# cbg-ethz/LongSom

Measured on AMD Instinct MI355X. Metric: genomic sites/s pileup+call, 10M-read BAM x 5k barcodes, 1/2/4/8 MI355X, higher is better.
Workload: dtype u32

## Files before the change

longsom_amd/csrc/call.hip:

```cpp
#include "lsg_ctx.h"
#include "call_rec.h"
#include "bb_tail.h"
#include <cstdio>
#include <cstring>
#include <cstdlib>
#include <hipcub/hipcub.hpp>

namespace lsg {

enum { CT_CAND = 0, CT_NCAND = 1, CT_HEADS = 4, CT_PASS = 6, CT_LIGHT = 16, CT_HEAVY = 32, CT_QTAIL = 48, CT_DEFER = 64, CT_WORDS = 80 };
struct CallArgs {
    const uint32_t* ne_units; const uint64_t* ne_mask; const uint32_t* ne_rowbase; const int2* ne_geom;
    uint32_t n_ne; int32_t n_ct;
    const uint32_t* rows[LSG_MAX_CELLTYPES]; uint64_t row_cap;
    const uint8_t* const* ref_ptr; const int64_t* contig_len;
    lsg_call_params p;
    double lgc0[2], lgcn[2];
    uint32_t* pass_list;
    const int16_t* tail_table;
    uint32_t* site_cnt; uint32_t* site_off;
    SiteRec* sites; CandCt* cands; uint64_t cand_cap;
    struct TailTask* light; struct TailTask* heavy; uint64_t task_cap;
    unsigned long long* counters;
    uint32_t arena_waves;
// ... 36 lines not shown
    const uint32_t up = n - k + 1;
    return k < up ? k : up;
}

__global__ void k_head_recs(CallArgs a) {
    const uint32_t i = blockIdx.x * blockDim.x + threadIdx.x;
    if (i >= (uint32_t)a.counters[CT_HEADS]) return;
    const uint32_t w = a.heads[i];
    const uint32_t tile = a.ne_units[w] / (uint32_t)a.n_ct;
    uint64_t mask[LSG_MAX_CELLTYPES] = {0, 0, 0, 0};
    uint32_t rbase[LSG_MAX_CELLTYPES] = {0, 0, 0, 0};
    for (uint32_t q = w; q < a.n_ne && q < w + (uint32_t)a.n_ct && a.ne_units[q] / (uint32_t)a.n_ct == tile; ++q) {
        const int ct = (int)(a.ne_units[q] % (uint32_t)a.n_ct);
        mask[ct] = a.ne_mask[q]; rbase[ct] = a.ne_rowbase[q];
    }
    const int2 geom = a.ne_geom[w];
    a.head_ref[i] = (uint64_t)(uintptr_t)a.ref_ptr[geom.y & 0xffffff];
    uint32_t* r = a.head_recs + (uint64_t)i * 16;
    r[0] = (uint32_t)a.contig_len[geom.y & 0xffffff]; r[1] = a.site_off[w]; r[2] = (uint32_t)geom.x; r[3] = (uint32_t)geom.y;
    for (int ct = 0; ct < LSG_MAX_CELLTYPES; ++ct) { r[4 + 2 * ct] = (uint32_t)mask[ct]; r[5 + 2 * ct] = (uint32_t)(mask[ct] >> 32); r[12 + ct] = rbase[ct]; }
}

constexpr int GATHER_WAVES = 4;
constexpr uint32_t CAND_CHUNK = 256, TASK_CHUNK = 64, HEAVY_CHUNK = 16;
template <int NCT>
__global__ __launch_bounds__(GATHER_WAVES * 64) __attribute__((amdgpu_waves_per_eu(NCT <= 2 ? 4 : 3))) void k_call_gather(CallArgs a) {
    const int lane = threadIdx.x & 63;
    const uint32_t wave = (uint32_t)__builtin_amdgcn_readfirstlane((int)(uint32_t)(((uint64_t)blockIdx.x * blockDim.x + threadIdx.x) >> 6));
    const uint32_t n_waves = (uint32_t)(((uint64_t)gridDim.x * blockDim.x) >> 6);
    const uint32_t n_heads = (uint32_t)a.counters[CT_HEADS];
    const uint32_t c_base = n_waves * CAND_CHUNK, l_base = n_waves * TASK_CHUNK, h_base = n_waves * HEAVY_CHUNK;
    uint32_t c_next = wave * CAND_CHUNK, c_end = c_next + CAND_CHUNK;
    uint32_t l_next = wave * TASK_CHUNK, l_end = l_next + TASK_CHUNK, h_next = wave * HEAVY_CHUNK, h_end = h_next + HEAVY_CHUNK;
    uint32_t n_cand_exact = 0;
    typedef uint32_t u32x16 __attribute__((ext_vector_type(16)));
    const __attribute__((address_space(4))) u32x16* H = (const __attribute__((address_space(4))) u32x16*)(uintptr_t)a.head_recs;
    const __attribute__((address_space(4))) uint64_t* HR = (const __attribute__((address_space(4))) uint64_t*)(uintptr_t)a.head_ref;
    u32x16 nxt = {};
    uint64_t ref_nxt = 0;
    if (wave < n_heads) { nxt = H[wave]; ref_nxt = HR[wave]; }
    for (uint32_t hi_ = wave; hi_ < n_heads; hi_ += n_waves) {
    const u32x16 rec = nxt;
    const uint8_t* ref = reinterpret_cast<const uint8_t*>((uintptr_t)ref_nxt);
    if (hi_ + n_waves < n_heads) { nxt = H[hi_ + n_waves]; ref_nxt = HR[hi_ + n_waves]; }
    uint64_t mask[NCT];
    uint32_t rbase[NCT];
    uint64_t any = 0;
#pragma unroll
    for (int ct = 0; ct < NCT; ++ct) { mask[ct] = (uint64_t)rec[4 + 2 * ct] | ((uint64_t)rec[5 + 2 * ct] << 32); rbase[ct] = rec[12 + ct]; any |= mask[ct]; }
    const bool site = (any >> lane) & 1ull;
    const uint64_t below = (1ull << lane) - 1ull;
    const uint64_t idx = (uint64_t)rec[1] + __popcll(any & below);
    const int2 geom = make_int2((int)rec[2], (int)rec[3]);
    const int tid = geom.y & 0xffffff;
    const int64_t pos = (int64_t)geom.x + lane;
    const int64_t clen = (int64_t)rec[0];
    const int64_t gx = (int64_t)geom.x;
    const int64_t xpos = lane < 5 ? gx - 5 + lane : gx + 59 + lane;
    const bool r0_ok = pos < clen, r1_ok = lane < 10 && xpos >= 0 && xpos < clen;
    const uint8_t r0_raw = ref[r0_ok ? pos : 0], r1_raw = ref[r1_ok ? xpos : 0];
    struct __attribute__((packed, aligned(4))) Quad { uint32_t x, y, z, w; };
    Quad q[NCT][4];
#pragma unroll
    for (int ct = 0; ct < NCT; ++ct) {
        const bool has_row = site && ((mask[ct] >> lane) & 1ull);
        const uint64_t row = has_row ? (uint64_t)(rbase[ct] & ~ROW_NARROW) + __popcll(mask[ct] & below) : (uint64_t)lane;
        const bool narrow = has_row && (rbase[ct] & ROW_NARROW);
        const char* R = reinterpret_cast<const char*>(a.rows[ct] + (row >> 6) * ROW_BLOCK_WORDS) + (narrow ? (row & 63) * 8 : (row & 63) * 16);
        const uint32_t stride = narrow ? 512u : 1024u;
#pragma unroll
        for (int k = 0; k < 4; ++k) q[ct][k] = *reinterpret_cast<const Quad*>(R + k * stride);
    }
    const uint8_t r0 = r0_ok ? r0_raw : (uint8_t)0, r1 = r1_ok ? r1_raw : (uint8_t)0;
    const uint8_t refb = site ? r0 : (uint8_t)'N';
    const int rsym = sym_of_ref(refb);
    const lsg_call_params& P = a.p;
    const int order[4] = {0, 1, 3, 2};
    uint32_t v_dp[NCT], v_nc[NCT], v_cc[NCT][6], v_bc[NCT][6];
#pragma unroll
    for (int ct = 0; ct < NCT; ++ct) {
        uint4 q0 = make_uint4(q[ct][0].x, q[ct][0].y, q[ct][0].z, q[ct][0].w), q1 = make_uint4(q[ct][1].x, q[ct][1].y, q[ct][1].z, q[ct][1].w);
        uint4 q2 = make_uint4(q[ct][2].x, q[ct][2].y, q[ct][2].z, q[ct][2].w), q3 = make_uint4(q[ct][3].x, q[ct][3].y, q[ct][3].z, q[ct][3].w);
        if (rbase[ct] & ROW_NARROW) {
            q0 = make_uint4(q0.x & 0xffffu, q0.x >> 16, q0.y & 0xffffu, q0.y >> 16); q1 = make_uint4(q1.x & 0xffffu, q1.x >> 16, q1.y & 0xffffu, q1.y >> 16);
            q2 = make_uint4(q2.x & 0xffffu, q2.x >> 16, q2.y & 0xffffu, q2.y >> 16); q3 = make_uint4(q3.x & 0xffffu, q3.x >> 16, q3.y & 0xffffu, q3.y >> 16);
        }
        v_dp[ct] = q0.x; v_nc[ct] = q0.y;
        v_cc[ct][0] = q0.z; v_cc[ct][1] = q0.w; v_cc[ct][2] = q1.x; v_cc[ct][3] = q1.y; v_cc[ct][4] = q1.z; v_cc[ct][5] = q1.w;
        v_bc[ct][0] = q2.z; v_bc[ct][1] = q2.w; v_bc[ct][2] = q3.x; v_bc[ct][3] = q3.y; v_bc[ct][4] = q3.z; v_bc[ct][5] = q3.w;
    }
    const uint32_t prev0 = (uint32_t)__shfl_up((int)r0, 1), prev1 = (uint32_t)__shfl_up((int)r1, 1), next0 = (uint32_t)__shfl_down((int)r0, 1);
    const uint64_t eq0 = __ballot(lane > 0 && r0 == (uint8_t)prev0), eq1 = __ballot(lane > 0 && lane != 5 && lane < 10 && r1 == (uint8_t)prev1);
    const uint32_t r1_4 = (uint32_t)__builtin_amdgcn_readlane((int)r1, 4), r1_5 = (uint32_t)__builtin_amdgcn_readlane((int)r1, 5);
    const uint32_t r0_0 = (uint32_t)__builtin_amdgcn_readlane((int)r0, 0), r0_63 = (uint32_t)__builtin_amdgcn_readlane((int)r0, 63);
    const uint64_t e_lo = (eq1 & 0x1eull) | ((uint64_t)(r0_0 == r1_4) << 5) | (eq0 << 5);
    const uint64_t e_hi = (eq0 >> 59) | ((uint64_t)(r1_5 == r0_63) << 5) | (((eq1 >> 6) & 0xfull) << 6);
    const uint64_t xlo = (e_lo >> 1) | (e_hi << 63), xhi = e_hi >> 1;
    const uint32_t xw = (uint32_t)((xlo >> lane) | (lane ? xhi << (64 - lane) : 0ull));
    const bool have_ctx = pos >= 5;
    int down_len = (int)((clen - (pos + 1)) < 5 ? (clen - (pos + 1)) : 5);
    if (down_len < 0) down_len = 0;
    const uint32_t ue = xw & 15u;
    const uint32_t de = down_len > 0 ? (xw >> 6) & ((1u << (down_len - 1)) - 1u) : 0u;
    auto longest = [](uint32_t m) { const uint32_t m2 = m & (m >> 1), m3 = m2 & (m >> 2), m4 = m3 & (m >> 3); return (int)((m != 0) + (m2 != 0) + (m3 != 0) + (m4 != 0)); };
    const int up_best = 1 + longest(ue), up_run = 1 + (int)__builtin_clz((((~ue) & 15u) << 28) | (1u << 27));
    const int dn_best = 1 + longest(de), dn_run = 1 + (int)__builtin_ctz((~de) | 16u);
    const uint8_t up4 = lane ? (uint8_t)prev0 : (uint8_t)r1_4, dn0 = lane < 63 ? (uint8_t)next0 : (uint8_t)r1_5;
    bool has_any = false, off_table = false;
    uint32_t n_light = 0, n_heavy = 0;
    int32_t s_alts_bc = 0, s_alts_cc = 0, s_dp = 0, s_nc = 0;
    if (site) {
#pragma unroll
        for (int ct = 0; ct < NCT; ++ct) {
            const uint32_t dp = v_dp[ct], nc = v_nc[ct];
            const bool ok = ((mask[ct] >> lane) & 1ull) && (int)dp >= P.min_cov && (int)nc >= P.min_cells;
            s_dp += ok ? (int32_t)dp : 0; s_nc += ok ? (int32_t)nc : 0;
#pragma unroll
            for (int s = 0; s < 6; ++s) {
                const bool nr = ok && s != rsym;
                const uint32_t b = nr ? v_bc[ct][s] : 0u, c = nr ? v_cc[ct][s] : 0u;
                const bool alt = s < 4 && b > 0;
                has_any |= alt;
                s_alts_bc += alt ? 0 : (int32_t)b; s_alts_cc += alt ? 0 : (int32_t)c;
                s_dp -= alt ? (int32_t)b : 0; s_nc -= alt ? (int32_t)c : 0;
                off_table |= alt && !(tail_in_table(b, dp) && tail_in_table(c, nc));
            }
        }
        if (s_alts_bc > 0) {
            off_table |= s_dp >= 0 && !tail_in_table((uint32_t)s_alts_bc, (uint32_t)s_dp);
            off_table |= s_nc >= 0 && s_alts_cc >= 0 && !tail_in_table((uint32_t)s_alts_cc, (uint32_t)s_nc);
        }
    }
    if (__ballot(off_table)) {
        if (site) {
#pragma unroll
            for (int ct = 0; ct < NCT; ++ct) {
                if (!((mask[ct] >> lane) & 1ull)) continue;
                const uint32_t dp = v_dp[ct], nc = v_nc[ct];
                if (!((int)dp >= P.min_cov && (int)nc >= P.min_cells)) continue;
#pragma unroll
                for (int s = 0; s < 4; ++s) {
                    const uint32_t b = v_bc[ct][s], c = v_cc[ct][s];
                    if (s == rsym || b == 0) continue;
                    if (!tail_in_table(b, dp)) { if (tail_work(b, dp) > 64) ++n_heavy; else ++n_light; }
                    if (!tail_in_table(c, nc)) { if (tail_work(c, nc) > 64) ++n_heavy; else ++n_light; }
                }
            }
            if (s_alts_bc > 0) {
                if (s_dp >= 0 && !tail_in_table((uint32_t)s_alts_bc, (uint32_t)s_dp)) { if (tail_work((uint32_t)s_alts_bc, (uint32_t)s_dp) > 64) ++n_heavy; else ++n_light; }
                if (s_nc >= 0 && s_alts_cc >= 0 && !tail_in_table((uint32_t)s_alts_cc, (uint32_t)s_nc)) { if (tail_work((uint32_t)s_alts_cc, (uint32_t)s_nc) > 64) ++n_heavy; else ++n_light; }
            }
        }
    }
    const unsigned long long cm = __ballot(has_any);
    uint32_t pl = n_light, ph = n_heavy, tot_l = 0, tot_h = 0;
    if (__ballot((n_light | n_heavy) != 0u)) {
        for (int o = 1; o < 64; o <<= 1) { const uint32_t vl = __shfl_up(pl, o), vh = __shfl_up(ph, o); if (lane >= o) { pl += vl; ph += vh; } }
        tot_l = __shfl(pl, 63); tot_h = __shfl(ph, 63);
    }
    const uint32_t n_c = (uint32_t)__popcll(cm);
    n_cand_exact += n_c;
    if (c_next + n_c > c_end) {
        uint32_t nb = 0;
        if (lane == 0) nb = (uint32_t)atomicAdd(&a.counters[CT_CAND], (unsigned long long)CAND_CHUNK) + c_base;
        c_next = (uint32_t)__builtin_amdgcn_readfirstlane((int)nb); c_end = c_next + CAND_CHUNK;
    }
    const uint32_t cbase = c_next; c_next += n_c;
    uint32_t l_old = l_next, l_room = l_end - l_next, l_new = 0;
    if (tot_l > l_room) {
        uint32_t nb = 0;
        if (lane == 0) nb = (uint32_t)atomicAdd(&a.counters[CT_LIGHT], (unsigned long long)TASK_CHUNK * ((tot_l - l_room + TASK_CHUNK - 1) / TASK_CHUNK)) + l_base;
        l_new = (uint32_t)__builtin_amdgcn_readfirstlane((int)nb);
        l_next = l_new + (tot_l - l_room); l_end = l_new + TASK_CHUNK * ((tot_l - l_room + TASK_CHUNK - 1) / TASK_CHUNK);
    } else l_next += tot_l;
    uint32_t h_old = h_next, h_room = h_end - h_next, h_new = 0;
    if (tot_h > h_room) {
        uint32_t nb = 0;
        if (lane == 0) nb = (uint32_t)atomicAdd(&a.counters[CT_HEAVY], (unsigned long long)HEAVY_CHUNK * ((tot_h - h_room + HEAVY_CHUNK - 1) / HEAVY_CHUNK)) + h_base;
        h_new = (uint32_t)__builtin_amdgcn_readfirstlane((int)nb);
        h_next = h_new + (tot_h - h_room); h_end = h_new + HEAVY_CHUNK * ((tot_h - h_room + HEAVY_CHUNK - 1) / HEAVY_CHUNK);
    } else h_next += tot_h;
    if (!site) continue;
    const uint32_t cand = cbase + (uint32_t)__popcll(cm & below);
    uint32_t li = pl - n_light, hi = ph - n_heavy;
    const int16_t* TT = a.tail_table;
    auto table_at = [&](uint32_t k, uint32_t n, int set) { return TT[tail_in_table(k, n) ? (uint32_t)set * TAIL_ENTRIES + tail_index(k, n) : 0u]; };
    int16_t t_bc[NCT][4], t_cc[NCT][4];
#pragma unroll
    for (int ct = 0; ct < NCT; ++ct) {
#pragma unroll
        for (int s = 0; s < 4; ++s) { t_bc[ct][s] = 0; t_cc[ct][s] = 0; }
    }
    if (cm) {
#pragma unroll
        for (int ct = 0; ct < NCT; ++ct) {
#pragma unroll
            for (int s = 0; s < 4; ++s) { t_bc[ct][s] = table_at(v_bc[ct][s], v_dp[ct], 0); t_cc[ct][s] = table_at(v_cc[ct][s], v_nc[ct], 1); }
        }
    }
    const int16_t t_nb = table_at((uint32_t)s_alts_bc, (uint32_t)s_dp, 0), t_nc = table_at((uint32_t)s_alts_cc, (uint32_t)s_nc, 1);
    auto emit_task = [&](uint32_t k, uint32_t n, int set, int16_t* dst, int16_t* loc, int16_t from_table) {
        if (tail_in_table(k, n)) { *loc = from_table; return; }
        TailTask t; t.k = k; t.n = n; t.dst = (uint64_t)dst | (uint64_t)set;
        if (tail_work(k, n) > 64) { const uint32_t p = hi < h_room ? h_old + hi : h_new + (hi - h_room); if (p < a.task_cap) a.heavy[p] = t; ++hi; }
        else { const uint32_t p = li < l_room ? l_old + li : l_new + (li - l_room); if (p < a.task_cap) a.light[p] = t; ++li; }
    };

    SiteRec sr;
    sr.key = ((int64_t)tid << 32) | pos; sr.ref = refb; sr.present = 0; sr.considered = 0; sr.has_cand = 0;
    sr.pad[0] = sr.pad[1] = sr.pad[2] = 0; sr.pad2 = 0; sr.cand = has_any ? cand : 0xFFFFFFFFu;
    sr.site_filter = 0;
    int n_considered = 0;
    bool alts_differ = false;
    uint32_t first_altset = 0; bool have_first = false;
    int lc_up = 0, lc_down = 0;
    SiteRec* srp = &a.sites[idx];
    const bool all_known = (n_light | n_heavy) == 0u;
    int f_pass = 0, f_nonsig = 0, f_with = 0; bool f_multi = false;

#pragma unroll
    for (int ct = 0; ct < NCT; ++ct) {
        CandCt cd;
        cd.n_alt = 0; cd.ct_filter = 0; cd.pad[0] = cd.pad[1] = 0;
#pragma unroll
        for (int q = 0; q < LSG_CALL_MAX_ALT; ++q) { cd.alt[q] = 0; cd.alt_bc[q] = 0; cd.alt_cc[q] = 0; cd.p_bc[q] = 0; cd.p_cc[q] = 0; }
        CandCt* cdp = has_any && cand < a.cand_cap ? &a.cands[(uint64_t)cand * NCT + ct] : nullptr;
        if ((mask[ct] >> lane) & 1ull) {
            sr.present |= (uint8_t)(1u << ct);
            const uint32_t dp = v_dp[ct], nc = v_nc[ct];
            if ((int)dp >= P.min_cov && (int)nc >= P.min_cells) {
                sr.considered |= (uint8_t)(1u << ct);
                ++n_considered;
                int na = 0; uint32_t altset = 0;
#pragma unroll
                for (int oi = 0; oi < 4; ++oi) {
                    const int s = order[oi];
                    const uint32_t b = v_bc[ct][s];
                    if (s == rsym || b == 0) continue;
                    const uint32_t c = v_cc[ct][s];
                    if (na < LSG_CALL_MAX_ALT) {
                        cd.alt[na] = (uint8_t)s; cd.alt_bc[na] = b; cd.alt_cc[na] = c;
                        if (cdp) { emit_task(b, dp, 0, &cdp->p_bc[na], &cd.p_bc[na], t_bc[ct][s]); emit_task(c, nc, 1, &cdp->p_cc[na], &cd.p_cc[na], t_cc[ct][s]); }
                    }
                    ++na; altset |= 1u << s;
                }
                cd.n_alt = (uint8_t)na;
                if (na > 0) {
                    sr.has_cand |= (uint8_t)(1u << ct);
                    if (!have_first) { first_altset = altset; have_first = true; } else if (altset != first_altset) alts_differ = true;
                    if (have_ctx) {
                        int first_s = -1, last_s = -1;
                        for (int oi = 0; oi < 4; ++oi) { const int s = order[oi]; if ((altset >> s) & 1u) { if (first_s < 0) first_s = s; last_s = s; } }
                        const int u = base_of_sym(first_s) == up4 ? up_run + 1 : 1;
                        const int ub = u > up_best ? u : up_best;
                        lc_up = ub > lc_up ? ub : lc_up;
                        int db = 1;
                        if (down_len > 0) { const int d = base_of_sym(last_s) == dn0 ? dn_run + 1 : 1; db = d > dn_best ? d : dn_best; }
                        lc_down = db > lc_down ? db : lc_down;
                    }
                }
            }
        }
        if (all_known && cd.n_alt > 0) {
            int32_t min_pbc = 100000, min_pcc = 100000;
#pragma unroll
            for (int q = 0; q < LSG_CALL_MAX_ALT; ++q) if (q < (int)cd.n_alt) { min_pbc = cd.p_bc[q] < min_pbc ? cd.p_bc[q] : min_pbc; min_pcc = cd.p_cc[q] < min_pcc ? cd.p_cc[q] : min_pcc; }
            uint8_t f;
            if (min_pbc >= 500 || min_pcc >= 500) f = LSG_CF_NONSIG;
            else if ((min_pbc > 10 && min_pbc < 500) || (min_pcc > 10 && min_pcc < 500)) f = LSG_CF_LOWSIG;
            else if (cd.n_alt > 1) f = LSG_CF_MULTI;
            else if ((int)cd.alt_cc[0] < P.min_ac_cells) f = LSG_CF_LOW_CELLS;
            else if ((int)cd.alt_bc[0] < P.min_ac_reads) f = LSG_CF_LOW_READS;
            else f = LSG_CF_PASS;
            cd.ct_filter = f;
            ++f_with; f_pass += f == LSG_CF_PASS; f_nonsig += f == LSG_CF_NONSIG; f_multi |= f == LSG_CF_MULTI;
        }
        if (cdp) *cdp = cd;
    }
    sr.cell_types_min = (uint8_t)n_considered;
    sr.sum_alts_bc = s_alts_bc; sr.sum_dp = s_dp; sr.sum_alts_cc = s_alts_cc; sr.sum_nc = s_nc;
    sr.noise_p_bc = -1; sr.noise_p_cc = -1;
    if (s_alts_bc > 0) {
        sr.noise_p_bc = -2; sr.noise_p_cc = -2;
        if (s_dp >= 0) emit_task((uint32_t)s_alts_bc, (uint32_t)s_dp, 0, &srp->noise_p_bc, &sr.noise_p_bc, t_nb);
        if (s_nc >= 0 && s_alts_cc >= 0) emit_task((uint32_t)s_alts_cc, (uint32_t)s_nc, 1, &srp->noise_p_cc, &sr.noise_p_cc, t_nc);
    }
    uint32_t sf = 0;
    if (sr.has_cand) {
        sf |= LSG_SF_CANDIDATE;
        if (alts_differ) sf |= LSG_SF_MULTI_ALLELIC;
        if (n_considered < P.min_cell_types) sf |= LSG_SF_MIN_CELL_TYPES;
        if (have_ctx && lc_up >= 4) sf |= LSG_SF_LC_UP;
        if (have_ctx && lc_down >= 4) sf |= LSG_SF_LC_DOWN;
    }
    bool pass_site = false;
    if (all_known) {
        const int32_t npb = sr.noise_p_bc, npc = sr.noise_p_cc;
        if (sr.has_cand) {
            if (f_pass > P.max_cell_types) sf |= LSG_SF_MULTIPLE_CELL_TYPES;
            if (f_multi) sf |= LSG_SF_MULTI_ALLELIC;
            if (f_with - f_pass - f_nonsig > 0) sf |= LSG_SF_CELL_TYPE_NOISE;
            if (s_alts_bc > 0 && ((npb >= 0 && npb < 500) || (npc >= 0 && npc < 500))) sf |= LSG_SF_NOISY_SITE;
            pass_site = sf == (uint32_t)LSG_SF_CANDIDATE && f_pass > 0;
        } else if (s_alts_bc > 0 && ((npb >= 0 && npb < 10) || (npc >= 0 && npc < 10))) sf |= LSG_SF_NOISY_SITE;
    }
    sr.site_filter = sf;
    *srp = sr;
    if (pass_site) {
        const unsigned long long q = atomicAdd(&a.counters[CT_PASS], 1ull);
        if (q < PASS_CAP) a.pass_list[q] = (uint32_t)idx;
    }
    const unsigned long long dm = __ballot(!all_known);
    if (dm) {
        unsigned long long q0 = 0;
        if (lane == __ffsll((long long)dm) - 1) q0 = atomicAdd(&a.counters[CT_DEFER], (unsigned long long)__popcll(dm));
        q0 = ((unsigned long long)(uint32_t)__shfl((int)(uint32_t)(q0 >> 32), __ffsll((long long)dm) - 1) << 32) | (uint32_t)__shfl((int)(uint32_t)q0, __ffsll((long long)dm) - 1);
        const unsigned long long q = q0 + __popcll(dm & below);
        if (!all_known && q < a.defer_cap) a.defer_list[q] = (uint32_t)idx;
    }
    }
    TailTask nul; nul.k = 0; nul.n = 0; nul.dst = 0;
    for (uint32_t p = l_next + (uint32_t)lane; p < l_end; p += 64) if (p < a.task_cap) a.light[p] = nul;
    for (uint32_t p = h_next + (uint32_t)lane; p < h_end; p += 64) if (p < a.task_cap) a.heavy[p] = nul;
    if (lane == 0 && n_cand_exact) atomicAdd(&a.counters[CT_NCAND], (unsigned long long)n_cand_exact);
}

__device__ __forceinline__ double tail_of_task(const TailTask& t, const CallArgs& a) {
    const int set = (int)(t.dst & 1ull);
    const double al = set ? a.p.alpha2 : a.p.alpha1, be = set ? a.p.beta2 : a.p.beta1;
    return bb_upper_tail(t.k, t.n, al, be, bb_pm0(t.n, al, be, a.lgc0[set]), a.lgcn[set]);
}

__global__ __launch_bounds__(256) void k_call_tails(CallArgs a) {
    const uint64_t n_all = a.counters[CT_LIGHT] + (uint64_t)a.arena_waves * TASK_CHUNK;
    const uint64_t n = n_all < a.task_cap ? n_all : a.task_cap;
    for (uint64_t i = (uint64_t)blockIdx.x * blockDim.x + threadIdx.x; i < n; i += (uint64_t)gridDim.x * blockDim.x) {
        const TailTask t = a.light[i];
        if (!(t.dst & ~1ull)) continue;
        *reinterpret_cast<int16_t*>(t.dst & ~1ull) = (int16_t)round4(tail_of_task(t, a));
    }
}

// ... 282 lines not shown
    uint32_t* heads = reinterpret_cast<uint32_t*>(a.counters + CT_WORDS);
    a.heads = heads;
    a.head_recs = reinterpret_cast<uint32_t*>((reinterpret_cast<uintptr_t>(heads + n_ne) + 63) & ~(uintptr_t)63);
    a.head_ref = reinterpret_cast<uint64_t*>(a.head_recs + (size_t)n_ne * 16);
    LSG_HIP(hipMemsetAsync(a.counters, 0, CT_WORDS * 8, st));
    hipLaunchKernelGGL(k_site_count, dim3((n_ne + 256) / 256), dim3(256), 0, st, a);
    size_t tb = 0;
    LSG_HIP(hipcub::DeviceScan::ExclusiveSum(nullptr, tb, a.site_cnt, a.site_off, (int)(n_ne + 1), st));
    if (c->d_cub_tmp.reserve(tb + 256)) return -1;
    tb = c->d_cub_tmp.cap;
    LSG_HIP(hipcub::DeviceScan::ExclusiveSum(c->d_cub_tmp.p, tb, a.site_cnt, a.site_off, (int)(n_ne + 1), st));
    {
        HasSites pred{a.site_cnt};
        hipcub::CountingInputIterator<uint32_t> it(0);
        uint32_t* d_nh = reinterpret_cast<uint32_t*>(a.counters + CT_HEADS);
        size_t tb2 = 0;
        LSG_HIP(hipcub::DeviceSelect::If(nullptr, tb2, it, heads, d_nh, (int)n_ne, pred, st));
        if (c->d_cub_tmp.reserve(tb2 + 256)) return -1;
        tb2 = c->d_cub_tmp.cap;
        LSG_HIP(hipcub::DeviceSelect::If(c->d_cub_tmp.p, tb2, it, heads, d_nh, (int)n_ne, pred, st));
    }
    hipLaunchKernelGGL(k_head_recs, dim3((n_ne + 255) / 256), dim3(256), 0, st, a);
    LSG_HIP(hipMemcpyAsync(c->h_pin, a.site_off + n_ne, 4, hipMemcpyDeviceToHost, st));
    LSG_HIP(hipStreamSynchronize(st));
    const uint32_t n_sites = *reinterpret_cast<const uint32_t*>(c->h_pin);
    if (n_sites > 0) {
        if (c->d_calls.reserve((size_t)n_sites * sizeof(SiteRec))) return -1;
        const unsigned gather_grid = (unsigned)(c->n_cus * 4);
        const uint64_t gather_waves = (uint64_t)gather_grid * GATHER_WAVES;
        if (c->ws[WS_CALL_CANDS].reserve(((size_t)n_sites + (size_t)2 * gather_waves * CAND_CHUNK) * sizeof(CandCt) * (size_t)c->n_ct)) return -1;
        a.arena_waves = (uint32_t)gather_waves;
        a.sites = c->d_calls.as<SiteRec>(); a.cands = c->ws[WS_CALL_CANDS].as<CandCt>(); a.cand_cap = n_sites + 2 * gather_waves * CAND_CHUNK;
        a.task_cap = (uint64_t)n_sites * (uint64_t)(8 * c->n_ct + 2);
        if (a.task_cap > (uint64_t)n_sites * tasks_per_site + 1024) a.task_cap = (uint64_t)n_sites * tasks_per_site + 1024;
        if (a.task_cap > 0x7fffffffull) a.task_cap = 0x7fffffffull;
        a.task_cap += gather_waves * TASK_CHUNK * 3;
        if (c->ws[WS_CALL_TASKS].reserve((size_t)a.task_cap * sizeof(TailTask) * 2)) return -1;
        a.light = c->ws[WS_CALL_TASKS].as<TailTask>(); a.heavy = a.light + a.task_cap;
        a.defer_cap = n_sites;
        if (c->d_defer_list.reserve((size_t)a.defer_cap * 4 + 64)) return -1;
        a.defer_list = c->d_defer_list.as<uint32_t>();
        switch (c->n_ct) {
            case 1: hipLaunchKernelGGL(k_call_gather<1>, dim3(gather_grid), dim3(GATHER_WAVES * 64), 0, st, a); break;
            case 2: hipLaunchKernelGGL(k_call_gather<2>, dim3(gather_grid), dim3(GATHER_WAVES * 64), 0, st, a); break;
            case 3: hipLaunchKernelGGL(k_call_gather<3>, dim3(gather_grid), dim3(GATHER_WAVES * 64), 0, st, a); break;
            default: hipLaunchKernelGGL(k_call_gather<4>, dim3(gather_grid), dim3(GATHER_WAVES * 64), 0, st, a); break;
        }
        hipLaunchKernelGGL(k_call_tails, dim3((unsigned)(c->n_cus * 16)), dim3(256), 0, st, a);
        hipLaunchKernelGGL(k_call_tails_heavy, dim3((unsigned)(c->n_cus * 8)), dim3(256), 0, st, a);
        hipLaunchKernelGGL(k_call_finish, dim3((unsigned)(c->n_cus * 2)), dim3(256), 0, st, a, n_sites);
        LSG_HIP(hipGetLastError());
// ... 102 lines not shown
```

Baseline: 3.328 billion.

## Compact candidate sites into per-wave LDS queue before per-site call processing

The gather kernel now writes non-candidate sites directly and pushes candidate sites into a per-wave shared-memory queue. Once 64 accumulate, or the tiles run out, it processes the queue with all lanes busy, so lanes no longer sit idle on sparse candidate tiles. Arena allocation and deferral are factored into helpers, and the gather grid is sized from the head count so each wave gets at least a minimum number of tiles. The cost is a large LDS footprint per block, which may reduce occupancy, plus an extra device-to-host copy of the head count.

```diff
diff --git a/longsom_amd/csrc/call.hip b/longsom_amd/csrc/call.hip
--- a/longsom_amd/csrc/call.hip
+++ b/longsom_amd/csrc/call.hip
@@ -82,9 +82,33 @@
 }
 
 constexpr int GATHER_WAVES = 4;
+constexpr uint32_t GATHER_MIN_TILES = 16;
 constexpr uint32_t CAND_CHUNK = 256, TASK_CHUNK = 64, HEAVY_CHUNK = 16;
+struct ArenaSpan {
+    uint32_t old, room, fresh;
+    __device__ __forceinline__ uint32_t at(uint32_t i) const { return i < room ? old + i : fresh + (i - room); }
+};
+__device__ __forceinline__ ArenaSpan arena_take(uint32_t& next, uint32_t& end, uint32_t tot, unsigned long long* counter, uint32_t base, uint32_t chunk, int lane) {
+    ArenaSpan s; s.old = next; s.room = end - next; s.fresh = 0;
+    if (tot > s.room) {
+        const uint32_t fresh_slots = chunk * ((tot - s.room + chunk - 1) / chunk);
+        uint32_t nb = 0;
+        if (lane == 0) nb = (uint32_t)atomicAdd(counter, (unsigned long long)fresh_slots) + base;
+        s.fresh = (uint32_t)__builtin_amdgcn_readfirstlane((int)nb);
+        next = s.fresh + (tot - s.room); end = s.fresh + fresh_slots;
+    } else next += tot;
+    return s;
+}
+template <int NCT>
+struct CandQueue {
+    uint32_t idx[64], pos[64], tid[64], ctx[64], edge[64], noise_p[64];
+    int32_t sum[4][64];
+    uint32_t dp[NCT][64], nc[NCT][64], bc[NCT][4][64], cc[NCT][4][64];
+};
 template <int NCT>
 __global__ __launch_bounds__(GATHER_WAVES * 64) __attribute__((amdgpu_waves_per_eu(NCT <= 2 ? 4 : 3))) void k_call_gather(CallArgs a) {
+    __shared__ CandQueue<NCT> queues[GATHER_WAVES];
+    CandQueue<NCT>& Q = queues[threadIdx.x >> 6];
     const int lane = threadIdx.x & 63;
     const uint32_t wave = (uint32_t)__builtin_amdgcn_readfirstlane((int)(uint32_t)(((uint64_t)blockIdx.x * blockDim.x + threadIdx.x) >> 6));
     const uint32_t n_waves = (uint32_t)(((uint64_t)gridDim.x * blockDim.x) >> 6);
@@ -93,13 +117,45 @@
     uint32_t c_next = wave * CAND_CHUNK, c_end = c_next + CAND_CHUNK;
     uint32_t l_next = wave * TASK_CHUNK, l_end = l_next + TASK_CHUNK, h_next = wave * HEAVY_CHUNK, h_end = h_next + HEAVY_CHUNK;
     uint32_t n_cand_exact = 0;
+    uint32_t qn = 0;
+    const lsg_call_params& P = a.p;
+    const uint64_t below = (1ull << lane) - 1ull;
+    const int16_t* TT = a.tail_table;
+    auto table_at = [&](uint32_t k, uint32_t n, int set) { return TT[tail_in_table(k, n) ? (uint32_t)set * TAIL_ENTRIES + tail_index(k, n) : 0u]; };
+    auto emit_task = [&](uint32_t k, uint32_t n, int set, int16_t* dst, int16_t* loc, int16_t from_table, const ArenaSpan& ls, const ArenaSpan& hs, uint32_t& li, uint32_t& hi) {
+        if (tail_in_table(k, n)) { *loc = from_table; return; }
+        TailTask t; t.k = k; t.n = n; t.dst = (uint64_t)dst | (uint64_t)set;
+        if (tail_work(k, n) > 64) { const uint32_t p = hs.at(hi); if (p < a.task_cap) a.heavy[p] = t; ++hi; }
+        else { const uint32_t p = ls.at(li); if (p < a.task_cap) a.light[p] = t; ++li; }
+    };
+    auto count_task = [](uint32_t k, uint32_t n, uint32_t& n_light, uint32_t& n_heavy) {
+        if (!tail_in_table(k, n)) { if (tail_work(k, n) > 64) ++n_heavy; else ++n_light; }
+    };
+    auto scan_tasks = [&](uint32_t& pl, uint32_t& ph, uint32_t& tot_l, uint32_t& tot_h) {
+        tot_l = 0; tot_h = 0;
+        if (__ballot((pl | ph) != 0u)) {
+            for (int o = 1; o < 64; o <<= 1) { const uint32_t vl = __shfl_up(pl, o), vh = __shfl_up(ph, o); if (lane >= o) { pl += vl; ph += vh; } }
+            tot_l = __shfl(pl, 63); tot_h = __shfl(ph, 63);
+        }
+    };
+    auto defer_sites = [&](bool mine, uint32_t site_idx) {
+        const unsigned long long dm = __ballot(mine);
+        if (dm) {
+            unsigned long long q0 = 0;
+            if (lane == __ffsll((long long)dm) - 1) q0 = atomicAdd(&a.counters[CT_DEFER], (unsigned long long)__popcll(dm));
+            q0 = ((unsigned long long)(uint32_t)__shfl((int)(uint32_t)(q0 >> 32), __ffsll((long long)dm) - 1) << 32) | (uint32_t)__shfl((int)(uint32_t)q0, __ffsll((long long)dm) - 1);
+            const unsigned long long q = q0 + __popcll(dm & below);
+            if (mine && q < a.defer_cap) a.defer_list[q] = site_idx;
+        }
+    };
     typedef uint32_t u32x16 __attribute__((ext_vector_type(16)));
     const __attribute__((address_space(4))) u32x16* H = (const __attribute__((address_space(4))) u32x16*)(uintptr_t)a.head_recs;
     const __attribute__((address_space(4))) uint64_t* HR = (const __attribute__((address_space(4))) uint64_t*)(uintptr_t)a.head_ref;
     u32x16 nxt = {};
     uint64_t ref_nxt = 0;
     if (wave < n_heads) { nxt = H[wave]; ref_nxt = HR[wave]; }
-    for (uint32_t hi_ = wave; hi_ < n_heads; hi_ += n_waves) {
+    for (uint32_t hi_ = wave; wave < n_heads && hi_ < n_heads + n_waves; hi_ += n_waves) {
+    const bool tile = hi_ < n_heads;
     const u32x16 rec = nxt;
     const uint8_t* ref = reinterpret_cast<const uint8_t*>((uintptr_t)ref_nxt);
     if (hi_ + n_waves < n_heads) { nxt = H[hi_ + n_waves]; ref_nxt = HR[hi_ + n_waves]; }
@@ -107,9 +163,8 @@
     uint32_t rbase[NCT];
     uint64_t any = 0;
 #pragma unroll
-    for (int ct = 0; ct < NCT; ++ct) { mask[ct] = (uint64_t)rec[4 + 2 * ct] | ((uint64_t)rec[5 + 2 * ct] << 32); rbase[ct] = rec[12 + ct]; any |= mask[ct]; }
+    for (int ct = 0; ct < NCT; ++ct) { mask[ct] = tile ? (uint64_t)rec[4 + 2 * ct] | ((uint64_t)rec[5 + 2 * ct] << 32) : 0ull; rbase[ct] = rec[12 + ct]; any |= mask[ct]; }
     const bool site = (any >> lane) & 1ull;
-    const uint64_t below = (1ull << lane) - 1ull;
     const uint64_t idx = (uint64_t)rec[1] + __popcll(any & below);
     const int2 geom = make_int2((int)rec[2], (int)rec[3]);
     const int tid = geom.y & 0xffffff;
@@ -134,8 +189,6 @@
     const uint8_t r0 = r0_ok ? r0_raw : (uint8_t)0, r1 = r1_ok ? r1_raw : (uint8_t)0;
     const uint8_t refb = site ? r0 : (uint8_t)'N';
     const int rsym = sym_of_ref(refb);
-    const lsg_call_params& P = a.p;
-    const int order[4] = {0, 1, 3, 2};
     uint32_t v_dp[NCT], v_nc[NCT], v_cc[NCT][6], v_bc[NCT][6];
 #pragma unroll
     for (int ct = 0; ct < NCT; ++ct) {
@@ -168,12 +221,15 @@
     const uint8_t up4 = lane ? (uint8_t)prev0 : (uint8_t)r1_4, dn0 = lane < 63 ? (uint8_t)next0 : (uint8_t)r1_5;
     bool has_any = false, off_table = false;
     uint32_t n_light = 0, n_heavy = 0;
+    uint32_t present = 0, considered = 0;
     int32_t s_alts_bc = 0, s_alts_cc = 0, s_dp = 0, s_nc = 0;
     if (site) {
 #pragma unroll
         for (int ct = 0; ct < NCT; ++ct) {
             const uint32_t dp = v_dp[ct], nc = v_nc[ct];
-            const bool ok = ((mask[ct] >> lane) & 1ull) && (int)dp >= P.min_cov && (int)nc >= P.min_cells;
+            const bool here = (mask[ct] >> lane) & 1ull;
+            const bool ok = here && (int)dp >= P.min_cov && (int)nc >= P.min_cells;
+            present |= here ? 1u << ct : 0u; considered |= ok ? 1u << ct : 0u;
             s_dp += ok ? (int32_t)dp : 0; s_nc += ok ? (int32_t)nc : 0;
 #pragma unroll
             for (int s = 0; s < 6; ++s) {
@@ -183,7 +239,6 @@
                 has_any |= alt;
                 s_alts_bc += alt ? 0 : (int32_t)b; s_alts_cc += alt ? 0 : (int32_t)c;
                 s_dp -= alt ? (int32_t)b : 0; s_nc -= alt ? (int32_t)c : 0;
-                off_table |= alt && !(tail_in_table(b, dp) && tail_in_table(c, nc));
             }
         }
         if (s_alts_bc > 0) {
@@ -192,192 +247,215 @@
         }
     }
     if (__ballot(off_table)) {
-        if (site) {
-#pragma unroll
-            for (int ct = 0; ct < NCT; ++ct) {
-                if (!((mask[ct] >> lane) & 1ull)) continue;
-                const uint32_t dp = v_dp[ct], nc = v_nc[ct];
-                if (!((int)dp >= P.min_cov && (int)nc >= P.min_cells)) continue;
-#pragma unroll
-                for (int s = 0; s < 4; ++s) {
-                    const uint32_t b = v_bc[ct][s], c = v_cc[ct][s];
-                    if (s == rsym || b == 0) continue;
-                    if (!tail_in_table(b, dp)) { if (tail_work(b, dp) > 64) ++n_heavy; else ++n_light; }
-                    if (!tail_in_table(c, nc)) { if (tail_work(c, nc) > 64) ++n_heavy; else ++n_light; }
-                }
-            }
-            if (s_alts_bc > 0) {
-                if (s_dp >= 0 && !tail_in_table((uint32_t)s_alts_bc, (uint32_t)s_dp)) { if (tail_work((uint32_t)s_alts_bc, (uint32_t)s_dp) > 64) ++n_heavy; else ++n_light; }
-                if (s_nc >= 0 && s_alts_cc >= 0 && !tail_in_table((uint32_t)s_alts_cc, (uint32_t)s_nc)) { if (tail_work((uint32_t)s_alts_cc, (uint32_t)s_nc) > 64) ++n_heavy; else ++n_light; }
-            }
-        }
-    }
+        if (site && s_alts_bc > 0) {
+            if (s_dp >= 0) count_task((uint32_t)s_alts_bc, (uint32_t)s_dp, n_light, n_heavy);
+            if (s_nc >= 0 && s_alts_cc >= 0) count_task((uint32_t)s_alts_cc, (uint32_t)s_nc, n_light, n_heavy);
+        }
+    }
+    const int16_t t_nb = table_at((uint32_t)s_alts_bc, (uint32_t)s_dp, 0), t_nc = table_at((uint32_t)s_alts_cc, (uint32_t)s_nc, 1);
     const unsigned long long cm = __ballot(has_any);
-    uint32_t pl = n_light, ph = n_heavy, tot_l = 0, tot_h = 0;
-    if (__ballot((n_light | n_heavy) != 0u)) {
-        for (int o = 1; o < 64; o <<= 1) { const uint32_t vl = __shfl_up(pl, o), vh = __shfl_up(ph, o); if (lane >= o) { pl += vl; ph += vh; } }
-        tot_l = __shfl(pl, 63); tot_h = __shfl(ph, 63);
-    }
     const uint32_t n_c = (uint32_t)__popcll(cm);
     n_cand_exact += n_c;
-    if (c_next + n_c > c_end) {
-        uint32_t nb = 0;
-        if (lane == 0) nb = (uint32_t)atomicAdd(&a.counters[CT_CAND], (unsigned long long)CAND_CHUNK) + c_base;
-        c_next = (uint32_t)__builtin_amdgcn_readfirstlane((int)nb); c_end = c_next + CAND_CHUNK;
-    }
-    const uint32_t cbase = c_next; c_next += n_c;
-    uint32_t l_old = l_next, l_room = l_end - l_next, l_new = 0;
-    if (tot_l > l_room) {
-        uint32_t nb = 0;
-        if (lane == 0) nb = (uint32_t)atomicAdd(&a.counters[CT_LIGHT], (unsigned long long)TASK_CHUNK * ((tot_l - l_room + TASK_CHUNK - 1) / TASK_CHUNK)) + l_base;
-        l_new = (uint32_t)__builtin_amdgcn_readfirstlane((int)nb);
-        l_next = l_new + (tot_l - l_room); l_end = l_new + TASK_CHUNK * ((tot_l - l_room + TASK_CHUNK - 1) / TASK_CHUNK);
-    } else l_next += tot_l;
-    uint32_t h_old = h_next, h_room = h_end - h_next, h_new = 0;
-    if (tot_h > h_room) {
-        uint32_t nb = 0;
-        if (lane == 0) nb = (uint32_t)atomicAdd(&a.counters[CT_HEAVY], (unsigned long long)HEAVY_CHUNK * ((tot_h - h_room + HEAVY_CHUNK - 1) / HEAVY_CHUNK)) + h_base;
-        h_new = (uint32_t)__builtin_amdgcn_readfirstlane((int)nb);
-        h_next = h_new + (tot_h - h_room); h_end = h_new + HEAVY_CHUNK * ((tot_h - h_room + HEAVY_CHUNK - 1) / HEAVY_CHUNK);
-    } else h_next += tot_h;
-    if (!site) continue;
-    const uint32_t cand = cbase + (uint32_t)__popcll(cm & below);
-    uint32_t li = pl - n_light, hi = ph - n_heavy;
-    const int16_t* TT = a.tail_table;
-    auto table_at = [&](uint32_t k, uint32_t n, int set) { return TT[tail_in_table(k, n) ? (uint32_t)set * TAIL_ENTRIES + tail_index(k, n) : 0u]; };
-    int16_t t_bc[NCT][4], t_cc[NCT][4];
-#pragma unroll
-    for (int ct = 0; ct < NCT; ++ct) {
-#pragma unroll
-        for (int s = 0; s < 4; ++s) { t_bc[ct][s] = 0; t_cc[ct][s] = 0; }
-    }
-    if (cm) {
+
+    uint32_t pl = n_light, ph = n_heavy, tot_l, tot_h;
+    scan_tasks(pl, ph, tot_l, tot_h);
+    const ArenaSpan ls = arena_take(l_next, l_end, tot_l, &a.counters[CT_LIGHT], l_base, TASK_CHUNK, lane);
+    const ArenaSpan hs = arena_take(h_next, h_end, tot_h, &a.counters[CT_HEAVY], h_base, HEAVY_CHUNK, lane);
+    const bool noise_known = (n_light | n_heavy) == 0u;
+    uint32_t w_ctx = 0, w_edge = 0, w_noise = 0;
+    if (site) {
+        uint32_t li = pl - n_light, hi = ph - n_heavy;
+        SiteRec* srp = &a.sites[idx];
+        int16_t noise_p_bc = -1, noise_p_cc = -1;
+        if (s_alts_bc > 0) {
+            noise_p_bc = -2; noise_p_cc = -2;
+            if (s_dp >= 0) emit_task((uint32_t)s_alts_bc, (uint32_t)s_dp, 0, &srp->noise_p_bc, &noise_p_bc, t_nb, ls, hs, li, hi);
+            if (s_nc >= 0 && s_alts_cc >= 0) emit_task((uint32_t)s_alts_cc, (uint32_t)s_nc, 1, &srp->noise_p_cc, &noise_p_cc, t_nc, ls, hs, li, hi);
+        }
+        if (has_any) {
+            w_ctx = (uint32_t)refb | present << 8 | considered << 12 | (uint32_t)have_ctx << 16 | (uint32_t)down_len << 17 | (uint32_t)up_best << 20 |
+                    (uint32_t)up_run << 23 | (uint32_t)dn_best << 26 | (uint32_t)dn_run << 29;
+            w_edge = (uint32_t)up4 | (uint32_t)dn0 << 8 | (uint32_t)noise_known << 16;
+            w_noise = (uint32_t)(uint16_t)noise_p_bc | (uint32_t)(uint16_t)noise_p_cc << 16;
+        } else {
+            SiteRec sr;
+            sr.key = ((int64_t)tid << 32) | pos; sr.ref = refb; sr.present = (uint8_t)present; sr.considered = (uint8_t)considered; sr.has_cand = 0;
+            sr.pad[0] = sr.pad[1] = sr.pad[2] = 0; sr.pad2 = 0; sr.cand = 0xFFFFFFFFu;
+            sr.cell_types_min = (uint8_t)__popc(considered);
+            sr.sum_alts_bc = s_alts_bc; sr.sum_dp = s_dp; sr.sum_alts_cc = s_alts_cc; sr.sum_nc = s_nc;
+            sr.noise_p_bc = noise_p_bc; sr.noise_p_cc = noise_p_cc;
+            const int32_t npb = noise_p_bc, npc = noise_p_cc;
+            sr.site_filter = noise_known && s_alts_bc > 0 && ((npb >= 0 && npb < 10) || (npc >= 0 && npc < 10)) ? (uint32_t)LSG_SF_NOISY_SITE : 0u;
+            *srp = sr;
+        }
+    }
+    defer_sites(site && !has_any && !noise_known, (uint32_t)idx);
+
+    if (qn + n_c > 64u || (!tile && qn)) {
+        asm volatile("" ::: "memory");
+        const bool live = (uint32_t)lane < qn;
+        const uint32_t e_ctx = live ? Q.ctx[lane] : (uint32_t)'N';
+        const uint8_t e_ref = (uint8_t)(e_ctx & 0xffu);
+        const int e_rsym = sym_of_ref(e_ref);
+        const uint32_t e_present = (e_ctx >> 8) & 15u, e_considered = (e_ctx >> 12) & 15u;
+        const bool e_have_ctx = (e_ctx >> 16) & 1u;
+        const int e_down_len = (int)((e_ctx >> 17) & 7u), e_up_best = (int)((e_ctx >> 20) & 7u), e_up_run = (int)((e_ctx >> 23) & 7u);
+        const int e_dn_best = (int)((e_ctx >> 26) & 7u), e_dn_run = (int)((e_ctx >> 29) & 7u);
+        int16_t t_bc[NCT][4], t_cc[NCT][4];
+        bool c_off = false;
+        uint32_t e_dp[NCT], e_nc[NCT], e_bc[NCT][4], e_cc[NCT][4];
 #pragma unroll
         for (int ct = 0; ct < NCT; ++ct) {
-#pragma unroll
-            for (int s = 0; s < 4; ++s) { t_bc[ct][s] = table_at(v_bc[ct][s], v_dp[ct], 0); t_cc[ct][s] = table_at(v_cc[ct][s], v_nc[ct], 1); }
-        }
-    }
-    const int16_t t_nb = table_at((uint32_t)s_alts_bc, (uint32_t)s_dp, 0), t_nc = table_at((uint32_t)s_alts_cc, (uint32_t)s_nc, 1);
-    auto emit_task = [&](uint32_t k, uint32_t n, int set, int16_t* dst, int16_t* loc, int16_t from_table) {
-        if (tail_in_table(k, n)) { *loc = from_table; return; }
-        TailTask t; t.k = k; t.n = n; t.dst = (uint64_t)dst | (uint64_t)set;
-        if (tail_work(k, n) > 64) { const uint32_t p = hi < h_room ? h_old + hi : h_new + (hi - h_room); if (p < a.task_cap) a.heavy[p] = t; ++hi; }
-        else { const uint32_t p = li < l_room ? l_old + li : l_new + (li - l_room); if (p < a.task_cap) a.light[p] = t; ++li; }
-    };
-
-    SiteRec sr;
-    sr.key = ((int64_t)tid << 32) | pos; sr.ref = refb; sr.present = 0; sr.considered = 0; sr.has_cand = 0;
-    sr.pad[0] = sr.pad[1] = sr.pad[2] = 0; sr.pad2 = 0; sr.cand = has_any ? cand : 0xFFFFFFFFu;
-    sr.site_filter = 0;
-    int n_considered = 0;
-    bool alts_differ = false;
-    uint32_t first_altset = 0; bool have_first = false;
-    int lc_up = 0, lc_down = 0;
-    SiteRec* srp = &a.sites[idx];
-    const bool all_known = (n_light | n_heavy) == 0u;
-    int f_pass = 0, f_nonsig = 0, f_with = 0; bool f_multi = false;
-
-#pragma unroll
-    for (int ct = 0; ct < NCT; ++ct) {
-        CandCt cd;
-        cd.n_alt = 0; cd.ct_filter = 0; cd.pad[0] = cd.pad[1] = 0;
-#pragma unroll
-        for (int q = 0; q < LSG_CALL_MAX_ALT; ++q) { cd.alt[q] = 0; cd.alt_bc[q] = 0; cd.alt_cc[q] = 0; cd.p_bc[q] = 0; cd.p_cc[q] = 0; }
-        CandCt* cdp = has_any && cand < a.cand_cap ? &a.cands[(uint64_t)cand * NCT + ct] : nullptr;
-        if ((mask[ct] >> lane) & 1ull) {
-            sr.present |= (uint8_t)(1u << ct);
-            const uint32_t dp = v_dp[ct], nc = v_nc[ct];
-            if ((int)dp >= P.min_cov && (int)nc >= P.min_cells) {
-                sr.considered |= (uint8_t)(1u << ct);
-                ++n_considered;
-                int na = 0; uint32_t altset = 0;
-#pragma unroll
-                for (int oi = 0; oi < 4; ++oi) {
-                    const int s = order[oi];
-                    const uint32_t b = v_bc[ct][s];
-                    if (s == rsym || b == 0) continue;
-                    const uint32_t c = v_cc[ct][s];
-                    if (na < LSG_CALL_MAX_ALT) {
-                        cd.alt[na] = (uint8_t)s; cd.alt_bc[na] = b; cd.alt_cc[na] = c;
-                        if (cdp) { emit_task(b, dp, 0, &cdp->p_bc[na], &cd.p_bc[na], t_bc[ct][s]); emit_task(c, nc, 1, &cdp->p_cc[na], &cd.p_cc[na], t_cc[ct][s]); }
-                    }
-                    ++na; altset |= 1u << s;
-                }
-                cd.n_alt = (uint8_t)na;
-                if (na > 0) {
-                    sr.has_cand |= (uint8_t)(1u << ct);
-                    if (!have_first) { first_altset = altset; have_first = true; } else if (altset != first_altset) alts_differ = true;
-                    if (have_ctx) {
-                        int first_s = -1, last_s = -1;
-                        for (int oi = 0; oi < 4; ++oi) { const int s = order[oi]; if ((altset >> s) & 1u) { if (first_s < 0) first_s = s; last_s = s; } }
-                        const int u = base_of_sym(first_s) == up4 ? up_run + 1 : 1;
-                        const int ub = u > up_best ? u : up_best;
-                        lc_up = ub > lc_up ? ub : lc_up;
-                        int db = 1;
-                        if (down_len > 0) { const int d = base_of_sym(last_s) == dn0 ? dn_run + 1 : 1; db = d > dn_best ? d : dn_best; }
-                        lc_down = db > lc_down ? db : lc_down;
+            e_dp[ct] = Q.dp[ct][lane]; e_nc[ct] = Q.nc[ct][lane];
+#pragma unroll
+            for (int s = 0; s < 4; ++s) { e_bc[ct][s] = Q.bc[ct][s][lane]; e_cc[ct][s] = Q.cc[ct][s][lane]; }
+        }
+#pragma unroll
+        for (int ct = 0; ct < NCT; ++ct) {
+            const uint32_t dp = live ? e_dp[ct] : 0u, nc = live ? e_nc[ct] : 0u;
+#pragma unroll
+            for (int s = 0; s < 4; ++s) {
+                const uint32_t b = live ? e_bc[ct][s] : 0u, c = live ? e_cc[ct][s] : 0u;
+                t_bc[ct][s] = table_at(b, dp, 0); t_cc[ct][s] = table_at(c, nc, 1);
+                const bool alt = ((e_considered >> ct) & 1u) && s != e_rsym && b > 0;
+                c_off |= alt && !(tail_in_table(b, dp) && tail_in_table(c, nc));
+            }
+        }
+        uint32_t c_light = 0, c_heavy = 0;
+        if (__ballot(c_off)) {
+            if (live) {
+#pragma unroll
+                for (int ct = 0; ct < NCT; ++ct) {
+                    if (!((e_considered >> ct) & 1u)) continue;
+#pragma unroll
+                    for (int s = 0; s < 4; ++s) {
+                        if (s == e_rsym || Q.bc[ct][s][lane] == 0) continue;
+                        count_task(Q.bc[ct][s][lane], Q.dp[ct][lane], c_light, c_heavy);
+                        count_task(Q.cc[ct][s][lane], Q.nc[ct][lane], c_light, c_heavy);
                     }
                 }
             }
         }
-        if (all_known && cd.n_alt > 0) {
-            int32_t min_pbc = 100000, min_pcc = 100000;
-#pragma unroll
-            for (int q = 0; q < LSG_CALL_MAX_ALT; ++q) if (q < (int)cd.n_alt) { min_pbc = cd.p_bc[q] < min_pbc ? cd.p_bc[q] : min_pbc; min_pcc = cd.p_cc[q] < min_pcc ? cd.p_cc[q] : min_pcc; }
-            uint8_t f;
-            if (min_pbc >= 500 || min_pcc >= 500) f = LSG_CF_NONSIG;
-            else if ((min_pbc > 10 && min_pbc < 500) || (min_pcc > 10 && min_pcc < 500)) f = LSG_CF_LOWSIG;
-            else if (cd.n_alt > 1) f = LSG_CF_MULTI;
-            else if ((int)cd.alt_cc[0] < P.min_ac_cells) f = LSG_CF_LOW_CELLS;
-            else if ((int)cd.alt_bc[0] < P.min_ac_reads) f = LSG_CF_LOW_READS;
-            else f = LSG_CF_PASS;
-            cd.ct_filter = f;
-            ++f_with; f_pass += f == LSG_CF_PASS; f_nonsig += f == LSG_CF_NONSIG; f_multi |= f == LSG_CF_MULTI;
-        }
-        if (cdp) *cdp = cd;
-    }
-    sr.cell_types_min = (uint8_t)n_considered;
-    sr.sum_alts_bc = s_alts_bc; sr.sum_dp = s_dp; sr.sum_alts_cc = s_alts_cc; sr.sum_nc = s_nc;
-    sr.noise_p_bc = -1; sr.noise_p_cc = -1;
-    if (s_alts_bc > 0) {
-        sr.noise_p_bc = -2; sr.noise_p_cc = -2;
-        if (s_dp >= 0) emit_task((uint32_t)s_alts_bc, (uint32_t)s_dp, 0, &srp->noise_p_bc, &sr.noise_p_bc, t_nb);
-        if (s_nc >= 0 && s_alts_cc >= 0) emit_task((uint32_t)s_alts_cc, (uint32_t)s_nc, 1, &srp->noise_p_cc, &sr.noise_p_cc, t_nc);
-    }
-    uint32_t sf = 0;
-    if (sr.has_cand) {
-        sf |= LSG_SF_CANDIDATE;
-        if (alts_differ) sf |= LSG_SF_MULTI_ALLELIC;
-        if (n_considered < P.min_cell_types) sf |= LSG_SF_MIN_CELL_TYPES;
-        if (have_ctx && lc_up >= 4) sf |= LSG_SF_LC_UP;
-        if (have_ctx && lc_down >= 4) sf |= LSG_SF_LC_DOWN;
-    }
-    bool pass_site = false;
-    if (all_known) {
-        const int32_t npb = sr.noise_p_bc, npc = sr.noise_p_cc;
-        if (sr.has_cand) {
-            if (f_pass > P.max_cell_types) sf |= LSG_SF_MULTIPLE_CELL_TYPES;
-            if (f_multi) sf |= LSG_SF_MULTI_ALLELIC;
-            if (f_with - f_pass - f_nonsig > 0) sf |= LSG_SF_CELL_TYPE_NOISE;
-            if (s_alts_bc > 0 && ((npb >= 0 && npb < 500) || (npc >= 0 && npc < 500))) sf |= LSG_SF_NOISY_SITE;
-            pass_site = sf == (uint32_t)LSG_SF_CANDIDATE && f_pass > 0;
-        } else if (s_alts_bc > 0 && ((npb >= 0 && npb < 10) || (npc >= 0 && npc < 10))) sf |= LSG_SF_NOISY_SITE;
-    }
-    sr.site_filter = sf;
-    *srp = sr;
-    if (pass_site) {
-        const unsigned long long q = atomicAdd(&a.counters[CT_PASS], 1ull);
-        if (q < PASS_CAP) a.pass_list[q] = (uint32_t)idx;
-    }
-    const unsigned long long dm = __ballot(!all_known);
-    if (dm) {
-        unsigned long long q0 = 0;
-        if (lane == __ffsll((long long)dm) - 1) q0 = atomicAdd(&a.counters[CT_DEFER], (unsigned long long)__popcll(dm));
-        q0 = ((unsigned long long)(uint32_t)__shfl((int)(uint32_t)(q0 >> 32), __ffsll((long long)dm) - 1) << 32) | (uint32_t)__shfl((int)(uint32_t)q0, __ffsll((long long)dm) - 1);
-        const unsigned long long q = q0 + __popcll(dm & below);
-        if (!all_known && q < a.defer_cap) a.defer_list[q] = (uint32_t)idx;
-    }
+        asm volatile("" ::: "memory");
+        uint32_t cpl = c_light, cph = c_heavy, ctot_l, ctot_h;
+        scan_tasks(cpl, cph, ctot_l, ctot_h);
+        const ArenaSpan cs = arena_take(c_next, c_end, qn, &a.counters[CT_CAND], c_base, CAND_CHUNK, lane);
+        const ArenaSpan cls = arena_take(l_next, l_end, ctot_l, &a.counters[CT_LIGHT], l_base, TASK_CHUNK, lane);
+        const ArenaSpan chs = arena_take(h_next, h_end, ctot_h, &a.counters[CT_HEAVY], h_base, HEAVY_CHUNK, lane);
+        const uint32_t e_idx = live ? Q.idx[lane] : 0u;
+        bool e_defer = false;
+        if (live) {
+            const uint32_t e_edge = Q.edge[lane], e_noise = Q.noise_p[lane];
+            const uint8_t e_up4 = (uint8_t)(e_edge & 0xffu), e_dn0 = (uint8_t)((e_edge >> 8) & 0xffu);
+            const uint32_t cand = cs.at((uint32_t)lane);
+            uint32_t cli = cpl - c_light, chi = cph - c_heavy;
+            const bool all_known = ((e_edge >> 16) & 1u) && (c_light | c_heavy) == 0u;
+            SiteRec sr;
+            sr.key = ((int64_t)Q.tid[lane] << 32) | (int64_t)Q.pos[lane]; sr.ref = e_ref; sr.present = (uint8_t)e_present; sr.considered = (uint8_t)e_considered; sr.has_cand = 0;
+            sr.pad[0] = sr.pad[1] = sr.pad[2] = 0; sr.pad2 = 0; sr.cand = cand;
+            const int n_considered = __popc(e_considered);
+            bool alts_differ = false;
+            uint32_t first_altset = 0; bool have_first = false;
+            int lc_up = 0, lc_down = 0;
+            int f_pass = 0, f_nonsig = 0, f_with = 0; bool f_multi = false;
+            const int order[4] = {0, 1, 3, 2};
+#pragma unroll
+            for (int ct = 0; ct < NCT; ++ct) {
+                CandCt cd;
+                cd.n_alt = 0; cd.ct_filter = 0; cd.pad[0] = cd.pad[1] = 0;
+#pragma unroll
+                for (int k = 0; k < LSG_CALL_MAX_ALT; ++k) { cd.alt[k] = 0; cd.alt_bc[k] = 0; cd.alt_cc[k] = 0; cd.p_bc[k] = 0; cd.p_cc[k] = 0; }
+                CandCt* cdp = cand < a.cand_cap ? &a.cands[(uint64_t)cand * NCT + ct] : nullptr;
+                if ((e_considered >> ct) & 1u) {
+                    const uint32_t dp = Q.dp[ct][lane], nc = Q.nc[ct][lane];
+                    int na = 0; uint32_t altset = 0;
+#pragma unroll
+                    for (int oi = 0; oi < 4; ++oi) {
+                        const int s = order[oi];
+                        const uint32_t b = Q.bc[ct][s][lane], c = Q.cc[ct][s][lane];
+                        const bool alt = s != e_rsym && b > 0;
+                        int16_t pb = 0, pc = 0;
+                        if (alt && cdp) { emit_task(b, dp, 0, &cdp->p_bc[na], &pb, t_bc[ct][s], cls, chs, cli, chi); emit_task(c, nc, 1, &cdp->p_cc[na], &pc, t_cc[ct][s], cls, chs, cli, chi); }
+#pragma unroll
+                        for (int k = 0; k < LSG_CALL_MAX_ALT; ++k)
+                            if (alt && k == na) { cd.alt[k] = (uint8_t)s; cd.alt_bc[k] = b; cd.alt_cc[k] = c; cd.p_bc[k] = pb; cd.p_cc[k] = pc; }
+                        na += alt; altset |= alt ? 1u << s : 0u;
+                    }
+                    cd.n_alt = (uint8_t)na;
+                    if (na > 0) {
+                        sr.has_cand |= (uint8_t)(1u << ct);
+                        if (!have_first) { first_altset = altset; have_first = true; } else if (altset != first_altset) alts_differ = true;
+                        if (e_have_ctx) {
+                            int first_s = -1, last_s = -1;
+                            for (int oi = 0; oi < 4; ++oi) { const int s = order[oi]; if ((altset >> s) & 1u) { if (first_s < 0) first_s = s; last_s = s; } }
+                            const int u = base_of_sym(first_s) == e_up4 ? e_up_run + 1 : 1;
+                            const int ub = u > e_up_best ? u : e_up_best;
+                            lc_up = ub > lc_up ? ub : lc_up;
+                            int db = 1;
+                            if (e_down_len > 0) { const int d = base_of_sym(last_s) == e_dn0 ? e_dn_run + 1 : 1; db = d > e_dn_best ? d : e_dn_best; }
+                            lc_down = db > lc_down ? db : lc_down;
+                        }
+                    }
+                }
+                if (all_known && cd.n_alt > 0) {
+                    int32_t min_pbc = 100000, min_pcc = 100000;
+#pragma unroll
+                    for (int k = 0; k < LSG_CALL_MAX_ALT; ++k) if (k < (int)cd.n_alt) { min_pbc = cd.p_bc[k] < min_pbc ? cd.p_bc[k] : min_pbc; min_pcc = cd.p_cc[k] < min_pcc ? cd.p_cc[k] : min_pcc; }
+                    uint8_t f;
+                    if (min_pbc >= 500 || min_pcc >= 500) f = LSG_CF_NONSIG;
+                    else if ((min_pbc > 10 && min_pbc < 500) || (min_pcc > 10 && min_pcc < 500)) f = LSG_CF_LOWSIG;
+                    else if (cd.n_alt > 1) f = LSG_CF_MULTI;
+                    else if ((int)cd.alt_cc[0] < P.min_ac_cells) f = LSG_CF_LOW_CELLS;
+                    else if ((int)cd.alt_bc[0] < P.min_ac_reads) f = LSG_CF_LOW_READS;
+                    else f = LSG_CF_PASS;
+                    cd.ct_filter = f;
+                    ++f_with; f_pass += f == LSG_CF_PASS; f_nonsig += f == LSG_CF_NONSIG; f_multi |= f == LSG_CF_MULTI;
+                }
+                if (cdp) *cdp = cd;
+            }
+            sr.cell_types_min = (uint8_t)n_considered;
+            sr.sum_alts_bc = Q.sum[0][lane]; sr.sum_dp = Q.sum[1][lane]; sr.sum_alts_cc = Q.sum[2][lane]; sr.sum_nc = Q.sum[3][lane];
+            sr.noise_p_bc = (int16_t)(e_noise & 0xffffu); sr.noise_p_cc = (int16_t)(e_noise >> 16);
+            uint32_t sf = LSG_SF_CANDIDATE;
+            if (alts_differ) sf |= LSG_SF_MULTI_ALLELIC;
+            if (n_considered < P.min_cell_types) sf |= LSG_SF_MIN_CELL_TYPES;
+            if (e_have_ctx && lc_up >= 4) sf |= LSG_SF_LC_UP;
+            if (e_have_ctx && lc_down >= 4) sf |= LSG_SF_LC_DOWN;
+            bool pass_site = false;
+            if (all_known) {
+                const int32_t npb = sr.noise_p_bc, npc = sr.noise_p_cc;
+                if (f_pass > P.max_cell_types) sf |= LSG_SF_MULTIPLE_CELL_TYPES;
+                if (f_multi) sf |= LSG_SF_MULTI_ALLELIC;
+                if (f_with - f_pass - f_nonsig > 0) sf |= LSG_SF_CELL_TYPE_NOISE;
+                if (sr.sum_alts_bc > 0 && ((npb >= 0 && npb < 500) || (npc >= 0 && npc < 500))) sf |= LSG_SF_NOISY_SITE;
+                pass_site = sf == (uint32_t)LSG_SF_CANDIDATE && f_pass > 0;
+            }
+            sr.site_filter = sf;
+            a.sites[e_idx] = sr;
+            if (pass_site) {
+                const unsigned long long k = atomicAdd(&a.counters[CT_PASS], 1ull);
+                if (k < PASS_CAP) a.pass_list[k] = e_idx;
+            }
+            e_defer = !all_known;
+        }
+        defer_sites(e_defer, e_idx);
+        qn = 0;
+        asm volatile("" ::: "memory");
+    }
+
+    if (has_any) {
+        const uint32_t slot = qn + (uint32_t)__popcll(cm & below);
+        Q.idx[slot] = (uint32_t)idx; Q.pos[slot] = (uint32_t)pos; Q.tid[slot] = (uint32_t)tid;
+        Q.ctx[slot] = w_ctx; Q.edge[slot] = w_edge; Q.noise_p[slot] = w_noise;
+        Q.sum[0][slot] = s_alts_bc; Q.sum[1][slot] = s_dp; Q.sum[2][slot] = s_alts_cc; Q.sum[3][slot] = s_nc;
+#pragma unroll
+        for (int ct = 0; ct < NCT; ++ct) {
+            Q.dp[ct][slot] = v_dp[ct]; Q.nc[ct][slot] = v_nc[ct];
+#pragma unroll
+            for (int s = 0; s < 4; ++s) { Q.bc[ct][s][slot] = v_bc[ct][s]; Q.cc[ct][s][slot] = v_cc[ct][s]; }
+        }
+    }
+    qn += n_c;
     }
     TailTask nul; nul.k = 0; nul.n = 0; nul.dst = 0;
     for (uint32_t p = l_next + (uint32_t)lane; p < l_end; p += 64) if (p < a.task_cap) a.light[p] = nul;
@@ -706,11 +784,14 @@
     }
     hipLaunchKernelGGL(k_head_recs, dim3((n_ne + 255) / 256), dim3(256), 0, st, a);
     LSG_HIP(hipMemcpyAsync(c->h_pin, a.site_off + n_ne, 4, hipMemcpyDeviceToHost, st));
+    LSG_HIP(hipMemcpyAsync(reinterpret_cast<char*>(c->h_pin) + 8, a.counters + CT_HEADS, 4, hipMemcpyDeviceToHost, st));
     LSG_HIP(hipStreamSynchronize(st));
     const uint32_t n_sites = *reinterpret_cast<const uint32_t*>(c->h_pin);
+    const uint32_t n_heads = *reinterpret_cast<const uint32_t*>(reinterpret_cast<const char*>(c->h_pin) + 8);
     if (n_sites > 0) {
         if (c->d_calls.reserve((size_t)n_sites * sizeof(SiteRec))) return -1;
-        const unsigned gather_grid = (unsigned)(c->n_cus * 4);
+        const unsigned gather_fill = (unsigned)((n_heads + GATHER_WAVES * GATHER_MIN_TILES - 1) / (GATHER_WAVES * GATHER_MIN_TILES));
+        const unsigned gather_grid = gather_fill < 1u ? 1u : gather_fill < (unsigned)(c->n_cus * 4) ? gather_fill : (unsigned)(c->n_cus * 4);
         const uint64_t gather_waves = (uint64_t)gather_grid * GATHER_WAVES;
         if (c->ws[WS_CALL_CANDS].reserve(((size_t)n_sites + (size_t)2 * gather_waves * CAND_CHUNK) * sizeof(CandCt) * (size_t)c->n_ct)) return -1;
         a.arena_waves = (uint32_t)gather_waves;
```

Result: no change. 3.305 billion (-0.7%).
